# CederGroupHub/smol

Hardware: AMD Instinct MI355X
Metric: attempted MC flips/s (node) + ns/flip/replica, 4096-site FCC canonical (higher is better)
Workload: dtype f64

## Files before the change

### smol_amd/csrc/mc_lean.h

```cpp
#pragma once
#include "smolmc_common.h"

template <int CTRL> __device__ __forceinline__ double dpp_xor_add(double v) {
    const int lo = __builtin_amdgcn_update_dpp(__double2loint(v), __double2loint(v), CTRL, 0xf, 0xf, true);
    const int hi = __builtin_amdgcn_update_dpp(__double2hiint(v), __double2hiint(v), CTRL, 0xf, 0xf, true);
    return v + __hiloint2double(hi, lo);
}
__device__ __forceinline__ double wave_sum_all(double v) {
    v = dpp_xor_add<0xB1>(v);
    v = dpp_xor_add<0x4E>(v);
    v = dpp_xor_add<0x141>(v);
    v = dpp_xor_add<0x140>(v);
    {
        const unsigned lo = (unsigned)__double2loint(v), hi = (unsigned)__double2hiint(v);
        const auto a = __builtin_amdgcn_permlane16_swap(lo, lo, false, false);
        const auto b = __builtin_amdgcn_permlane16_swap(hi, hi, false, false);
        v = __hiloint2double((int)b[0], (int)a[0]) + __hiloint2double((int)b[1], (int)a[1]);
    }
    {
        const unsigned lo = (unsigned)__double2loint(v), hi = (unsigned)__double2hiint(v);
        const auto a = __builtin_amdgcn_permlane32_swap(lo, lo, false, false);
        const auto b = __builtin_amdgcn_permlane32_swap(hi, hi, false, false);
        v = __hiloint2double((int)b[0], (int)a[0]) + __hiloint2double((int)b[1], (int)a[1]);
    }
    return v;
}

template <int CTRL> __device__ __forceinline__ float dpp_add_f32(float v) {
    const int t = __builtin_amdgcn_update_dpp(0, __float_as_int(v), CTRL, 0xf, 0xf, true);
    return v + __int_as_float(t);
}
__device__ __forceinline__ float wave_sum_f32_uniform(float v) {
    v = dpp_add_f32<0xB1>(v);
    v = dpp_add_f32<0x4E>(v);
    v = dpp_add_f32<0x141>(v);
    v = dpp_add_f32<0x140>(v);
    float total;
    asm volatile("s_nop 1\n\t"
                 "v_add_f32_dpp %1, %1, %1 row_bcast:15 row_mask:0xa bank_mask:0xf\n\t"
                 "s_nop 1\n\t"
                 "v_add_f32_dpp %1, %1, %1 row_bcast:31 row_mask:0xc bank_mask:0xf\n\t"
                 "s_nop 1\n\t"
                 "v_readlane_b32 %0, %1, 63\n\t"
                 "s_nop 1"
                 : "=s"(total), "+v"(v));
    return total;
}
__device__ __forceinline__ float wave_sum_f32_lane63(float v) {
    v = dpp_add_f32<0xB1>(v);
    v = dpp_add_f32<0x4E>(v);
    v = dpp_add_f32<0x141>(v);
    v = dpp_add_f32<0x140>(v);
    asm volatile("s_nop 1\n\t"
                 "v_add_f32_dpp %0, %0, %0 row_bcast:15 row_mask:0xa bank_mask:0xf\n\t"
                 "s_nop 1\n\t"
                 "v_add_f32_dpp %0, %0, %0 row_bcast:31 row_mask:0xc bank_mask:0xf"
                 : "+v"(v));
    return v;
}

__device__ __forceinline__ double lean_ewald_partial(const LeanParams &P, const uint8_t *occ, int lane,
                                                     int s, int swa, int swm, int swb) {
    const double *g = P.ew_G + (size_t)s * P.ew_nact;
    const int W = P.ew_W, na = P.ew_nact;
    double out = 0;
    for (int j0 = lane; j0 < na; j0 += 64 * 8) {
        int k[8];
        double gk[8], q[8];
#pragma unroll
        for (int u = 0; u < 8; ++u) {
            const int jj = min(j0 + 64 * u, na - 1);
            k[u] = P.ew_act[jj];
            gk[u] = g[jj];
        }
#pragma unroll
        for (int u = 0; u < 8; ++u)
            q[u] = P.ew_qs[(size_t)k[u] * W + (int)occ[lean_swz(k[u], swa, swm, swb)]];
#pragma unroll
        for (int u = 0; u < 8; ++u)
            out = fma((j0 + 64 * u < na && k[u] != s) ? q[u] : 0.0, gk[u], out);
    }
    return out;
}

template <int FOOT = 2, bool PRE = false>
__device__ __forceinline__ void field_apply(const LeanParams &P, double *phi, int lane, int s, double dq,
                                            const uint32_t (&e0)[27], const bool have_e0) {
    const int js = s - P.sbase;
    const double keep = phi[js];
    const LeanParamsKernarg Q = rare_params();
    const unsigned char *gx = (const unsigned char *)Q->ew_gx;
    if (gx != nullptr) {
        const uint32_t *E8 = Q->ew_E8;
        const uint32_t s8[1] = {Q->ew_S8[js]};
        const double d[1] = {dq};
        if (PRE && have_e0) field_sweep_gx_pre27(phi, E8, gx, lane, P.ew_nact, s8, d, e0);
        else field_sweep_gx_multi<1, FOOT>(phi, E8, gx, lane, P.ew_nact, s8, d);
    } else {
        const double *g = P.ew_G + (size_t)s * P.ew_nact;
        field_sweep<false>(phi, g, g, lane, P.ew_nact, dq, 0.0);
    }
    phi[js] = keep;
}

template <int FOOT = 2>
__device__ __forceinline__ void field_apply(const LeanParams &P, double *phi, int lane, int s, double dq) {
    const uint32_t none[27] = {};
    field_apply<FOOT, false>(P, phi, lane, s, dq, none, false);
}

template <int FOOT = 1, bool FEW = false>
__device__ __forceinline__ void field_apply_flips(double *phi, int lane, int nfl, int vsite, double vdq) {
    const LeanParamsKernarg Q = rare_params();

    const unsigned char *gx = (const unsigned char *)Q->ew_gx;
    auto site_of = [&](int f) { return (int)rdlane((uint32_t)vsite, f); };
    auto dq_of = [&](int f) {
        return __hiloint2double((int)rdlane((uint32_t)__double2hiint(vdq), f), (int)rdlane((uint32_t)__double2loint(vdq), f));
    };
    const int sb = Q->sbase, na = Q->ew_nact;
    if (gx == nullptr) {
        const double *G = Q->ew_G;
        for (int f = 0; f < nfl; ++f) {
            const double dqf = dq_of(f);
            if (dqf == 0.0) continue;
            const double *g = G + (size_t)site_of(f) * na;
            field_sweep<false>(phi, g, g, lane, na, dqf, 0.0);
        }
        return;
    }
    const uint32_t *E8 = Q->ew_E8, *S8 = Q->ew_S8;
    for (int f0 = 0; f0 < nfl; f0 += 4) {
        const int n = min(4, nfl - f0);
        uint32_t s8[4];
        double dq[4];
#pragma unroll
        for (int k = 0; k < 4; ++k) {
            const int f = k < n ? f0 + k : f0;
            s8[k] = S8[site_of(f) - sb];
            dq[k] = k < n ? dq_of(f) : 0.0;
        }
        if (FEW && n <= 3) {
            const uint32_t a[3] = {s8[0], s8[1], s8[2]};
            const double d[3] = {dq[0], dq[1], dq[2]};
            field_sweep_gx_multi<3, FOOT>(phi, E8, gx, lane, na, a, d);
        } else if (n == 1) {
            const uint32_t a[1] = {s8[0]};
            const double d[1] = {dq[0]};
            field_sweep_gx_multi<1, FOOT>(phi, E8, gx, lane, na, a, d);
        } else if (n == 2) {
            const uint32_t a[2] = {s8[0], s8[1]};
            const double d[2] = {dq[0], dq[1]};
            field_sweep_gx_multi<2, FOOT>(phi, E8, gx, lane, na, a, d);
        } else if (n == 3) {
// ... 155 lines not shown
    static_assert(KF == 0 || (!WL && !BIAS && !SOLO), "correlation-function tables: plain Metropolis layouts only");
    static_assert(!REPLAY || (!WL && OCC == 0), "replay: Metropolis variants (Wang-Landau: mc_wl_kernel)");
    constexpr int NACC = KF ? KF : 1;
    constexpr int EWM = EWX & 3;
    constexpr bool WMU = (EWX & 4) != 0;
    static_assert(!WMU || (HAS_MU && !WL && !REPLAY), "per-walker chemical potentials: semigrand Metropolis variants");
    constexpr bool ROWS = lean_rows(MM);
    constexpr int MMX = lean_mm_max(MM);
    constexpr bool STRAIGHT = ROWS && STEP == SMOLMC_STEP_SWAP && OCC == 0 && !HAS_MU;
    constexpr int TAIL_AHEAD = (STRAIGHT && MM == 21) ? 1 : 0;
    static_assert(!ROWS || (SOLO && NSLOT == 2 && EWX == 0 && !REPLAY && KF == 0 && !WL && !BIAS), "solo rows: plain Metropolis, solo layout");
    constexpr bool HAS_EW = EWM != 0, ew_field = EWM == 2;
    extern __shared__ __attribute__((aligned(16))) unsigned char smem[];
    if ((uint32_t)(uintptr_t)smem != 0u) __builtin_trap();
    const int lane = threadIdx.x & 63;
    const int wave = SOLO ? 0 : threadIdx.x >> 6;
    const int nwaves = SOLO ? 1 : blockDim.x >> 6;
    const int r = uni(blockIdx.x * nwaves + wave);
    const size_t per_wave = (size_t)P.Nlds + 64 * 8 + (WL ? (size_t)P.wl.L * 24 : 0) +
                            ((HAS_EW && ew_field) ? 64 + (size_t)P.ew_nact * 8 : 0);
    double *s_dt = SOLO ? (double *)(smem + ((per_wave + 15) & ~(size_t)15)) : (double *)smem;
    const uint32_t dt_off = SOLO ? (uint32_t)((per_wave + 15) & ~(size_t)15) : 0u;
    double *s_mu = s_dt + P.dt_len;
    double *s_q = s_mu + 8, *s_dg = s_mu + 16;
    unsigned char *wbase = SOLO ? smem : (unsigned char *)(s_mu + 24) + (size_t)wave * per_wave;
    uint8_t *occ = wbase;
    double *s_feat = (double *)(wbase + P.Nlds);
    double *wl_S = s_feat + 64;
    long long *wl_Hh = (long long *)(wl_S + (WL ? P.wl.L : 0));
    long long *wl_Oc = wl_Hh + (WL ? P.wl.L : 0);
    double *phi = (double *)(wbase + P.Nlds + 64 * 8 + 64);
    const int swa = P.swz_a, swm = P.swz_m, swb = P.swz_b;
    for (int i = threadIdx.x; i < P.dt_len; i += blockDim.x) s_dt[i] = P.dt[i];
    if (HAS_MU && !WMU && threadIdx.x < 8) s_mu[threadIdx.x] = threadIdx.x < P.ncodes ? P.mu_row[threadIdx.x] : 0.0;
    if (WMU) {
        s_mu = (double *)(smem + P.mu_cell_off) + uni(wave * 8);
        if (lane < 8 && r < P.R) s_mu[lane] = lane < P.ncodes ? P.mu_row[(size_t)r * 8 + lane] : 0.0;
    }
    if (HAS_EW && ew_field && threadIdx.x < 8) {
        s_q[threadIdx.x] = P.ew_qrow[threadIdx.x];
        s_dg[threadIdx.x] = P.ew_dgrow[threadIdx.x];
    }
    const bool live = r < P.R;
    if (live) {
        const uint32_t *src = (const uint32_t *)(P.occ + (size_t)r * P.Npad);
        for (int i = lane; i < P.Npad / 4; i += 64)
            *(uint32_t *)(occ + lean_swz(4 * i, swa, swm, swb)) = src[i];
        s_feat[lane] = (WL && lane < P.F) ? P.features[(size_t)r * P.F + lane] : 0.0;
        if (HAS_EW && ew_field)
            for (int j = lane; j < P.ew_nact; j += 64) phi[j] = P.ew_phi[(size_t)r * P.ew_nact + j];
        if (WL)
            for (int i = lane; i < P.wl.L; i += 64) {
                wl_S[i] = P.wl.entropy[(size_t)r * P.wl.L + i];
                wl_Hh[i] = P.wl.hist[(size_t)r * P.wl.L + i];
                wl_Oc[i] = P.wl.occur[(size_t)r * P.wl.L + i];
            }
    }
    __syncthreads();
    if (!live) return;

    constexpr bool EPRE = HAS_EW && STEP == SMOLMC_STEP_FLIP && !REPLAY;
    uint32_t ereg[27] = {};
    bool epre_on = false;
    if (EPRE) {
        const LeanParamsKernarg Q = rare_params();
        const uint32_t *E8 = Q->ew_E8;
        epre_on = ew_field && Q->ew_gx != nullptr && (Q->ew_nact >> 6) >= 27;
        if (epre_on) {
#pragma unroll
            for (int u = 0; u < 27; ++u) ereg[u] = E8[64 * u + lane];
        }
    }

    uint32_t doff8[NSLOT], st8[NSLOT][MMX], sfeat[NSLOT];
    double wgt[NSLOT], acc[NSLOT], sfs[NSLOT];
    double accK[NSLOT][NACC];
    uint32_t kslot[NSLOT];
#pragma unroll
    for (int it = 0; it < NSLOT; ++it) {
        const LeanSlot sl = P.slots[it * 64 + lane];
        doff8[it] = sl.doff8 + dt_off;
        sfeat[it] = sl.feat;
        sfs[it] = sl.live ? sl.fs : 0.0;
        kslot[it] = sl.live;
#pragma unroll
        for (int m = 0; m < (ROWS ? lean_mm_of(MM, it) : MM); ++m) st8[it][m] = sl.stride8[m];
        wgt[it] = sl.w;
        acc[it] = 0.0;
#pragma unroll
        for (int k = 0; k < NACC; ++k) accK[it][k] = 0.0;
    }
    const int wl_stride = WL ? P.F : 64;
    const int wl_k = WL ? max(1, min(8, 63 / max(wl_stride, 1))) : 1;
    uint32_t sfeat_wl[NSLOT];
#pragma unroll
    for (int it = 0; it < NSLOT; ++it) sfeat_wl[it] = sfeat[it] + (uint32_t)((lane % wl_k) * wl_stride);
    int wl_rd[8];
#pragma unroll
    for (int k = 0; k < 8; ++k) wl_rd[k] = (WL && k < wl_k && lane < wl_stride) ? lane + k * wl_stride : 63;
    auto wl_cur_feat = [&]() -> double {
        const int f = lane < wl_stride ? lane : 0;
        double t[8];
#pragma unroll
        for (int k = 0; k < 8; ++k) t[k] = k < wl_k ? s_feat[f + (k < wl_k ? k : 0) * wl_stride] : 0.0;
        return ((t[0] + t[1]) + (t[2] + t[3])) + ((t[4] + t[5]) + (t[6] + t[7]));
    };
    auto reduce_features = [&](double *dst) {
#pragma unroll
        for (int it = 0; it < NSLOT; ++it) {
            if (KF == 0) {
                __hip_atomic_fetch_add(&dst[sfeat[it]], sfs[it] * acc[it], __ATOMIC_RELAXED,
                                       __HIP_MEMORY_SCOPE_WAVEFRONT);
            } else {
#pragma unroll
                for (int k = 0; k < NACC; ++k) {
                    const bool on = (uint32_t)k < kslot[it];
                    __hip_atomic_fetch_add(&dst[sfeat[it] + (on ? k : 0)], on ? sfs[it] * accK[it][k] : 0.0,
                                           __ATOMIC_RELAXED, __HIP_MEMORY_SCOPE_WAVEFRONT);
                }
            }
        }
    };
    double H = P.enthalpy[r];
    const double nbeta = WL ? 0.0 : -P.beta[r];
    double wl_m = WL ? P.wl.m[r] : 0.0;
    double wl_bq = WL ? floordiv_exact(H - P.wl.vmin, P.wl.bin) : 0.0;
    const double wl_inv_bin = WL ? 1.0 / P.wl.bin : 0.0;
    long long wl_counter = WL ? P.wl.counter[r] : 0;
    long long wl_rem_check = WL ? (P.wl.check ? wl_counter % P.wl.check : 1) : 0;
    unsigned long long step = P.nsteps[r];
    uint32_t nacc_add = 0;
    const uint32_t key0 = (uint32_t)P.seeds[r], key1 = (uint32_t)(P.seeds[r] >> 32);
    const uint32_t nact = (uint32_t)P.nact, nt8 = P.nt8, snt8 = P.snt8;
    const int sbase = P.sbase;
    double acc_mu = 0.0, acc_ew = 0.0;
    const int btype = BIAS ? P.bias_type : 0;
    const int brows = (btype && btype != SMOLMC_BIAS_FUGACITY) ? P.bias_rows : 0;
    double bias_acc = 0.0, chg[SMOLMC_MAX_BIAS_ROWS];
#pragma unroll
    for (int k = 0; k < SMOLMC_MAX_BIAS_ROWS; ++k) chg[k] = k < brows ? P.charge[(size_t)r * SMOLMC_MAX_BIAS_ROWS + k] : 0.0;
    constexpr bool FAST = !WL && !HAS_EW;
    float thr_lo = 0.0f, thr_hi = 0.0f;
    const double inv_nbeta = FAST ? 1.0 / nbeta : 0.0;
    uint32_t nacc_before = 0;
    int nsite = 0, naddr = 0;
    double *featp = P.features + (size_t)r * P.F;
    const double base_feat = lane < P.F ? featp[lane] : 0.0;
    uint32_t smp_countdown = P.smp.every ? (uint32_t)P.smp.every : 0xffffffffu;
    long long smp_index = 0;
    uint32_t W0 = 0;
    int cand[4] = {0, 0, 0, 0}, canda[4] = {0, 0, 0, 0};
    double vGc = 0.0;
    double logu = 0.0;
    unsigned long long batch64_base = ~0ull;
    unsigned long long batch_base = ~0ull;
    constexpr int ROW = lean_row_len(MM, NSLOT);
    constexpr int NW = SOLO ? ROW : ROW / 2;
    constexpr uint32_t ENT = SOLO ? 4u : 2u;
    constexpr uint32_t SITE_BYTES = 64u * ROW * ENT;
    const __amdgpu_buffer_rsrc_t idx_rs = __builtin_amdgcn_make_buffer_rsrc(
        SOLO ? (void *)P.idx32 : (void *)P.idx, 0, 0x7fffffff, 0x00020000);
    const uint32_t lane_voff = (uint32_t)lane * (ROW * ENT);

    int s1, a1;
    RowWords<NW> row1;
    uint32_t ridx = 0;
    double lu_rp = 0.0;
    int rp_bad = 0;
    auto rp_site = [&](const uint32_t i) -> int {
        const int v = uni(P.rp_steps[((size_t)r * (uint32_t)P.steps + i) * 4]);
        return v >= 0 ? v : sbase;
    };
    {
        if (REPLAY) {
            s1 = rp_site(0u);
        } else {
            const unsigned long long sp = step - 1ull;
            const uint32_t w = (uint32_t)uni((int)philox4x32_10((uint32_t)sp, (uint32_t)(sp >> 32), 0u, 0u,
                                                                key0, key1).w[1]);
            s1 = sbase + (int)__umulhi(w, nact);
        }
        a1 = lean_swz(s1, swa, swm, swb);
        row1 = load_row<NW>(idx_rs, lane_voff, (uint32_t)(ROWS ? a1 : s1) * SITE_BYTES);
    }

    double *wl_pend = WL ? P.wl.meanf + (size_t)r * P.wl.L * P.F : nullptr;
    double wl_pc[8] = {0.0, 0.0, 0.0, 0.0, 0.0, 0.0, 0.0, 0.0};
    auto wl_pend_sum = [&]() -> double {
        return ((wl_pc[0] + wl_pc[1]) + (wl_pc[2] + wl_pc[3])) + ((wl_pc[4] + wl_pc[5]) + (wl_pc[6] + wl_pc[7]));
    };
    uint32_t steps_left = (uint32_t)P.steps;
    while (steps_left != 0u) {
        const unsigned long long base = step & ~15ull;
        if (!REPLAY && base != batch_base) {
            batch_base = base;
            const unsigned long long st = base + (unsigned)(lane >> 2);
            const philox_out o = philox4x32_10((uint32_t)st, (uint32_t)(st >> 32), (uint32_t)(lane & 3),
                                               0u, key0, key1);
            W0 = o.w[0];
            nsite = sbase + (int)__umulhi(o.w[1], nact);
            naddr = lean_swz(nsite, swa, swm, swb);
            if ((step & ~63ull) != batch64_base) {
                batch64_base = step & ~63ull;
                const unsigned long long s64 = batch64_base + (unsigned)lane;
                const philox_out a = philox4x32_10((uint32_t)s64, (uint32_t)(s64 >> 32), 0u, 0u, key0, key1);
                logu = log(philox_u53(a.w[2], a.w[3]));
                if (FAST) {
                    const double thr = logu * inv_nbeta;
                    const double eps = P.fast_eps + 1e-6 * fabs(thr);
                    thr_lo = P.fast_eps > 0.0 ? (float)(thr - eps) : -INFINITY;
                    thr_hi = P.fast_eps > 0.0 ? (float)(thr + eps) : INFINITY;
                }
            }
            if (STEP == SMOLMC_STEP_SWAP) {
                cand[0] = sbase + (int)__umulhi(o.w[0], nact);
                cand[1] = sbase + (int)__umulhi(o.w[1], nact);
                cand[2] = sbase + (int)__umulhi(o.w[2], nact);
                cand[3] = sbase + (int)__umulhi(o.w[3], nact);
#pragma unroll
                for (int j = 0; j < 4; ++j) canda[j] = lean_swz(cand[j], swa, swm, swb);
                if (HAS_EW && ew_field) {
                    const int prev = __shfl(nsite, (lane & ~3) - 4);
                    const int site_l = lane < 4 ? s1 : prev;
                    vGc = P.ew_G[(size_t)cand[0] * P.ew_nact + (site_l - sbase)];
                }
            }
        }
        uint32_t chunk = 16u - (uint32_t)(step & 15ull);
        chunk = min(chunk, steps_left);
        chunk = min(chunk, smp_countdown);
        steps_left -= chunk;
        smp_countdown -= chunk;
        const unsigned long long chunk_end = step + chunk;
        int l4 = (int)(step & 15ull) * 4;
        int l64 = (int)(step & 63ull);
        float tlo_s = 0.0f, thi_s = 0.0f;
        uint32_t va2 = 0u, okm = 0u;
        do {
        __builtin_amdgcn_s_setprio(1);
        int s1n, a1n;
        int rq1 = 0, rq2 = -1, rq3 = 0;
        bool rp_empty = false;
        if (REPLAY) {
            const int *rec = P.rp_steps + ((size_t)r * (uint32_t)P.steps + ridx) * 4;
            const int q0 = uni(rec[0]);
            rq1 = uni(rec[1]); rq2 = uni(rec[2]); rq3 = uni(rec[3]);
            rp_empty = q0 < 0;
            double u = uni_d(P.rp_u[(size_t)r * (uint32_t)P.steps + ridx]);
            if (u != u) u = 0.0;
            lu_rp = log(u);
            s1n = ridx + 1u < (uint32_t)P.steps ? rp_site(ridx + 1u) : s1;
            a1n = lean_swz(s1n, swa, swm, swb);
            if (FAST) {
                const double thr = lu_rp * inv_nbeta, eps = P.fast_eps + 1e-6 * fabs(thr);
                thr_lo = P.fast_eps > 0.0 ? (float)(thr - eps) : -INFINITY;
                thr_hi = P.fast_eps > 0.0 ? (float)(thr + eps) : INFINITY;
            }
        } else {
            s1n = (int)rdlane((uint32_t)nsite, l4);
            a1n = (int)rdlane((uint32_t)naddr, l4);
        }
        if constexpr (STRAIGHT) {
            tlo_s = __uint_as_float(rdlane(__float_as_uint(thr_lo), l64));
            thi_s = __uint_as_float(rdlane(__float_as_uint(thr_hi), l64));
        }
        uint32_t va1 = (uint32_t)a1;
        asm volatile("" : "+v"(va1));
        const int vo1 = (int)occ_ld<SOLO>(occ, va1);
        const int o1 = uni(vo1);
        int nfl, s2, a2, n1, n2 = 0, o2 = 0;
        if (STEP != SMOLMC_STEP_SWAP) { s2 = s1; a2 = a1; }
        int fb = -1;
        if (REPLAY) {
            if (STEP == SMOLMC_STEP_FLIP) {
                nfl = rp_empty ? 0 : 1;
                n1 = rp_empty ? o1 : rq1;
                rp_bad |= (rq2 >= 0) ? 1 : 0;
            } else if (!rp_empty && rq2 >= 0) {
                nfl = 2;
                s2 = rq2;
                a2 = lean_swz(s2, swa, swm, swb);
                o2 = uni((int)occ_ld<SOLO>(occ, (uint32_t)a2));
                n2 = rq3;
                n1 = rq1;
                rp_bad |= (n2 != o1 || n1 != o2) ? 1 : 0;
                n2 = o1; n1 = o2;
            } else {
                nfl = 0; s2 = s1; a2 = a1; o2 = o1; n2 = o1; n1 = o1;
                rp_bad |= (!rp_empty || rq2 >= 0) ? 1 : 0;
            }
        } else if (STEP == SMOLMC_STEP_FLIP) {
            const uint32_t kk = __umulhi(rdlane(W0, l4 + 1), (uint32_t)(P.ncodes - 1));
            n1 = (int)kk + ((int)kk >= o1 ? 1 : 0);
            nfl = 1;
        } else {
            nfl = 2;
            n2 = o1;
#define SMOLMC_CAND_MASK(J)                                                                        \
    const int v##J = (int)occ_ld<SOLO>(occ, (uint32_t)canda[J]);                                   \
    const unsigned long long m##J = __ballot(v##J != o1) & (0xEull << l4);
#define SMOLMC_CAND_TAKE(J)                                                                        \
    {                                                                                              \
        const int b = __ffsll((long long)m##J) - 1;                                                \
        s2 = (int)rdlane((uint32_t)cand[J], b);                                                    \
        a2 = (int)rdlane((uint32_t)canda[J], b);                                                   \
        o2 = (int)rdlane((uint32_t)v##J, b);                                                       \
        if (J == 0) fb = b;                                                                        \
    }
            SMOLMC_CAND_MASK(0)
            if constexpr (STRAIGHT) {
                unsigned long long mt = m0;
                uint32_t ta = (uint32_t)canda[0];
                int tv = v0;
                if (__builtin_expect(m0 == 0ull, 0)) {
                    SMOLMC_CAND_MASK(1)
                    mt = m1; ta = (uint32_t)canda[1]; tv = v1;
                    if (m1 == 0ull) {
                        SMOLMC_CAND_MASK(2)
                        mt = m2; ta = (uint32_t)canda[2]; tv = v2;
                        if (m2 == 0ull) {
                            SMOLMC_CAND_MASK(3)
                            mt = m3; ta = (uint32_t)canda[3]; tv = v3;
                            if (m3 == 0ull) {
                                mt = 1ull; ta = va1; tv = o1; nfl = 0;
                                const unsigned long long cur = chunk_end - chunk;
                                for (uint32_t q = 0;; ++q) {
                                    const philox_out o = philox4x32_10((uint32_t)cur, (uint32_t)(cur >> 32),
                                                                       4u + 64u * q + (uint32_t)lane, 0u, key0, key1);
                                    int selsite = -1, selv = 0;
#pragma unroll
                                    for (int j = 3; j >= 0; --j) {
                                        const int cs = sbase + (int)__umulhi(o.w[j], nact);
                                        const int v = (int)occ[lean_swz(cs, swa, swm, swb)];
                                        if (v != o1) { selsite = lean_swz(cs, swa, swm, swb); selv = v; }
                                    }
                                    const unsigned long long m = __ballot(selsite >= 0);
                                    if (m) {
                                        const int b = __ffsll((long long)m) - 1;
                                        ta = rdlane((uint32_t)selsite, b);
                                        tv = (int)rdlane((uint32_t)selv, b);
                                        nfl = 2;
                                        break;
                                    }
                                    if ((q & 63u) == 0) {
                                        int any = 0;
                                        for (uint32_t a = lane; a < nact; a += 64)
                                            any |= ((int)occ[lean_swz(sbase + (int)a, swa, swm, swb)] != o1);
                                        if (__ballot(any) == 0ull) break;
                                    }
                                }
                            }
                        }
                    }
                }
                const int b = __ffsll((long long)mt) - 1;
                a2 = (int)rdlane(ta, b);
                o2 = (int)rdlane((uint32_t)tv, b);
                s2 = a2;
            } else
            if (m0) SMOLMC_CAND_TAKE(0)
            else {
                SMOLMC_CAND_MASK(1)
                if (m1) SMOLMC_CAND_TAKE(1)
                else {
                    SMOLMC_CAND_MASK(2)
                    if (m2) SMOLMC_CAND_TAKE(2)
                    else {
                        SMOLMC_CAND_MASK(3)
                        if (m3) SMOLMC_CAND_TAKE(3)
                        else {
                            bool hit = false;
                            const unsigned long long cur = chunk_end - chunk;
                            for (uint32_t q = 0;; ++q) {
                                const philox_out o = philox4x32_10((uint32_t)cur, (uint32_t)(cur >> 32),
                                                                   4u + 64u * q + (uint32_t)lane, 0u, key0, key1);
                                int selsite = -1, selv = 0;
#pragma unroll
                                for (int j = 3; j >= 0; --j) {
                                    const int cs = sbase + (int)__umulhi(o.w[j], nact);
                                    const int v = (int)occ[lean_swz(cs, swa, swm, swb)];
                                    if (v != o1) { selsite = ROWS ? lean_swz(cs, swa, swm, swb) : cs; selv = v; }
                                }
                                const unsigned long long m = __ballot(selsite >= 0);
                                if (m) {
                                    const int b = __ffsll((long long)m) - 1;
                                    s2 = (int)rdlane((uint32_t)selsite, b);
                                    a2 = ROWS ? s2 : lean_swz(s2, swa, swm, swb);
                                    o2 = (int)rdlane((uint32_t)selv, b);
                                    hit = true;
                                    break;
                                }
                                if ((q & 63u) == 0) {
                                    int any = 0;
                                    for (uint32_t a = lane; a < nact; a += 64)
                                        any |= ((int)occ[lean_swz(sbase + (int)a, swa, swm, swb)] != o1);
                                    if (__ballot(any) == 0ull) break;
                                }
                            }
                            if (!hit) { nfl = 0; s2 = s1; a2 = a1; o2 = o1; }
                        }
                    }
                }
            }
#undef SMOLMC_CAND_MASK
#undef SMOLMC_CAND_TAKE
            n1 = o2;
        }

        __builtin_amdgcn_s_setprio(2);
        RowWords<NW> row2 = row1;
        if (STEP == SMOLMC_STEP_SWAP) {
            row2 = load_row<NW>(idx_rs, lane_voff, (uint32_t)(ROWS ? a2 : s2) * SITE_BYTES);
        }
        if (WL) {
            unsafeAtomicAdd(wl_pend + lane, wl_pend_sum());
        }

        constexpr bool DIFF = STEP == SMOLMC_STEP_SWAP;
        double e = 0.0, d1[NSLOT], d2[NSLOT];
        uint32_t dp[NSLOT];
        uint32_t ad1[NSLOT], ad2[NSLOT];
        {
            const uint32_t pair1 = (uint32_t)o1 * snt8 + (uint32_t)n1 * nt8;
#pragma unroll
            for (int it = 0; it < NSLOT; ++it) {
                uint32_t a = doff8[it];
                if (DIFF) a = dp[it] = doff8[it] + pair1;
#pragma unroll
                for (int m = 0; m < (ROWS ? lean_mm_of(MM, it) : MM); ++m) a += __umul24(st8[it][m], (uint32_t)occ_ld<SOLO>(occ, bounded(row_addr<SOLO, NW>(row1, (ROWS ? lean_row_off(MM, it) : it * MM) + m), (uint32_t)P.Nlds)));
                if (DIFF) {
                    d1[it] = SMOLMC_LDS_F64(a);
                    if (KF) ad1[it] = a;
                } else {
                    d1[it] = SMOLMC_LDS_F64(a + pair1);
                    if (KF) ad1[it] = a + pair1;
                    e = fma(wgt[it], d1[it], e);
                }
            }
        }
        row1 = load_row<NW>(idx_rs, lane_voff, (uint32_t)(ROWS ? a1n : s1n) * SITE_BYTES);
        double ew_part = 0.0, ew_uni = 0.0;
        double dq1 = 0.0, dq2 = 0.0;
        if (HAS_EW) {
            if (ew_field) {
                dq1 = s_q[n1] - s_q[o1];
                ew_uni = 2.0 * dq1 * phi[s1 - sbase] + (s_dg[n1] - s_dg[o1]);
            } else {
                const int W = P.ew_W;
                dq1 = P.ew_qs[(size_t)s1 * W + n1] - P.ew_qs[(size_t)s1 * W + o1];
                ew_part = 2.0 * dq1 * lean_ewald_partial(P, occ, lane, s1, swa, swm, swb);
                ew_uni = 2.0 * dq1 * P.ew_frozen[s1] +
                         (P.ew_dg[(size_t)s1 * W + n1] - P.ew_dg[(size_t)s1 * W + o1]);
            }
        }
        if (STEP == SMOLMC_STEP_SWAP) {
            occ_st<SOLO>(occ, va1, (uint8_t)n1);
            const uint32_t pair2 = (uint32_t)o2 * snt8 + (uint32_t)n2 * nt8;
            if constexpr (TAIL_AHEAD != 0) {
                uint32_t g[NSLOT][MMX];
#pragma unroll
                for (int it = 0; it < NSLOT; ++it) {
#pragma unroll
                    for (int m = 0; m < lean_mm_of(MM, it); ++m) g[it][m] = (uint32_t)occ_ld<SOLO>(occ, bounded(row_addr<SOLO, NW>(row2, lean_row_off(MM, it) + m), (uint32_t)P.Nlds));
                }
                __builtin_amdgcn_sched_barrier(0);
                l4 = (int)opaque_u32((uint32_t)l4 + 4u);
                l64 = (int)opaque_u32((uint32_t)l64 + 1u);
                chunk = opaque_u32(chunk - 1u);
                va2 = (uint32_t)a2;
                asm volatile("" : "+v"(va2));
                __builtin_amdgcn_sched_barrier(0);
#pragma unroll
                for (int it = 0; it < NSLOT; ++it) {
                    uint32_t a = dp[it];
#pragma unroll
                    for (int m = 0; m < lean_mm_of(MM, it); ++m) a += __umul24(st8[it][m], g[it][m]);
                    d1[it] -= SMOLMC_LDS_F64(a);
                    e = fma(wgt[it], d1[it], e);
                }
            } else
#pragma unroll
            for (int it = 0; it < NSLOT; ++it) {
                uint32_t a = DIFF ? dp[it] : doff8[it];
#pragma unroll
                for (int m = 0; m < (ROWS ? lean_mm_of(MM, it) : MM); ++m) a += __umul24(st8[it][m], (uint32_t)occ_ld<SOLO>(occ, bounded(row_addr<SOLO, NW>(row2, (ROWS ? lean_row_off(MM, it) : it * MM) + m), (uint32_t)P.Nlds)));
                if (DIFF) {
                    d1[it] -= SMOLMC_LDS_F64(a);
                    if (KF) ad2[it] = a;
                    e = fma(wgt[it], d1[it], e);
                } else {
                    d2[it] = SMOLMC_LDS_F64(a + pair2);
                    if (KF) ad2[it] = a + pair2;
                    e = fma(wgt[it], d2[it], e);
                }
            }
            if (HAS_EW) {
                if (ew_field) {
                    dq2 = s_q[n2] - s_q[o2];
                    const double cross =
                        fb >= 0 ? __hiloint2double((int)rdlane((uint32_t)__double2hiint(vGc), fb),
                                                   (int)rdlane((uint32_t)__double2loint(vGc), fb))
                                : P.ew_G[(size_t)s2 * P.ew_nact + (s1 - sbase)];
                    ew_uni += 2.0 * dq2 * (phi[s2 - sbase] + dq1 * cross) + (s_dg[n2] - s_dg[o2]);
                } else {
                    const int W = P.ew_W;
                    dq2 = P.ew_qs[(size_t)s2 * W + n2] - P.ew_qs[(size_t)s2 * W + o2];
                    ew_part += 2.0 * dq2 * lean_ewald_partial(P, occ, lane, s2, swa, swm, swb);
                    ew_uni += 2.0 * dq2 * P.ew_frozen[s2] +
                              (P.ew_dg[(size_t)s2 * W + n2] - P.ew_dg[(size_t)s2 * W + o2]);
                }
            }
        }
        double dMu = 0.0;
        if (HAS_MU && nfl >= 1) {
            dMu = s_mu[n1] - s_mu[o1];
            if (nfl == 2) dMu += s_mu[n2] - s_mu[o2];
        }
        double dH = 0.0, dEw = 0.0;
        double wl_nbq = 0.0;
        double dB = 0.0, dQ[SMOLMC_MAX_BIAS_ROWS] = {0.0, 0.0, 0.0, 0.0};
        if (btype && nfl >= 1) {
            if (btype == SMOLMC_BIAS_FUGACITY) {
                dB = P.bias_pair[o1 * 8 + n1];
                if (nfl == 2) dB += P.bias_pair[o2 * 8 + n2];
            } else {
                double sq_new = 0.0, sq_old = 0.0;
#pragma unroll
                for (int k = 0; k < SMOLMC_MAX_BIAS_ROWS; ++k)
                    if (k < brows) {
                        const double *bp = P.bias_pair + k * P.bias_row_stride;
                        double x = bp[o1 * 8 + n1];
                        if (nfl == 2) x += bp[o2 * 8 + n2];
                        dQ[k] = x;
                        const double cn = chg[k] + x;
                        sq_old += chg[k] * chg[k];
                        sq_new += cn * cn;
                    }
                dB = -P.bias_pen * sq_new - (-P.bias_pen * sq_old);
            }
        }
        auto exact_decision = [&]() -> bool {
            dH = wave_sum_all(e);
            if (HAS_EW) {
                dEw = (ew_field ? 0.0 : wave_sum_all(ew_part)) + ew_uni;
                dH += P.ew_coef * dEw;
            }
            if (HAS_MU) dH -= dMu;
            const double lu = REPLAY ? lu_rp
                                     : __hiloint2double((int)rdlane((uint32_t)__double2hiint(logu), l64 - TAIL_AHEAD),
                                                        (int)rdlane((uint32_t)__double2loint(logu), l64 - TAIL_AHEAD));
            if (!WL) {
                const double exponent = nbeta * dH + 0.0 + dB;
                return __ballot((exponent >= 0.0) || (exponent > lu)) != 0ull;
            } else {
                const double new_h = H + dH;
                if (new_h < P.wl.vmin || new_h >= P.wl.vmax) {
                    return false;
                } else {
                    const int b = (int)wl_bq;
                    wl_nbq = floordiv_exact_inv(new_h - P.wl.vmin, P.wl.bin, wl_inv_bin);
                    const int nb = (int)wl_nbq;
                    const double exponent = wl_S[b] - wl_S[nb] + 0.0;
                    return __ballot((exponent >= 0.0) || (exponent > lu)) != 0ull;
                }
            }
        };
        constexpr bool SELACC = DIFF && FAST && !BIAS;
        uint32_t sel_hi = 0u;
        auto on_accept = [&]() {
            if (KF) {
                const unsigned char *kb = (const unsigned char *)P.dtk;
#pragma unroll
                for (int it = 0; it < NSLOT; ++it) {
                    const uint32_t g1 = doff8[it] * (uint32_t)(SMOLMC_LEAN_MAX_KF - 1) + ad1[it];
                    const uint32_t g2 = doff8[it] * (uint32_t)(SMOLMC_LEAN_MAX_KF - 1) + ad2[it];
#pragma unroll
                    for (int k = 0; k < NACC; ++k) {
                        const bool on = (uint32_t)k < kslot[it];
                        const uint32_t off = (uint32_t)k * P.ktab8;
                        double v = on ? *(const double *)(kb + (g1 + off)) : 0.0;
                        if (STEP == SMOLMC_STEP_SWAP) {
                            const double v2 = on ? *(const double *)(kb + (g2 + off)) : 0.0;
                            v = DIFF ? v - v2 : v + v2;
                        }
                        accK[it][k] += v;
                    }
                }
            }
            if (SELACC) {
                sel_hi = 0x3ff00000u;
            } else if (!WL) {
#pragma unroll
                for (int it = 0; it < NSLOT; ++it) acc[it] += d1[it];
                if (STEP == SMOLMC_STEP_SWAP && !DIFF) {
#pragma unroll
                    for (int it = 0; it < NSLOT; ++it) acc[it] += d2[it];
                }
            } else {
#pragma unroll
                for (int it = 0; it < NSLOT; ++it) {
                    const double dd = (STEP == SMOLMC_STEP_SWAP && !DIFF) ? d1[it] + d2[it] : d1[it];
                    __hip_atomic_fetch_add(&s_feat[sfeat_wl[it]], sfs[it] * dd, __ATOMIC_RELAXED,
                                           __HIP_MEMORY_SCOPE_WAVEFRONT);
                }
            }
            if (STEP == SMOLMC_STEP_FLIP) occ_st<SOLO>(occ, va1, (uint8_t)n1);
            if (STEP == SMOLMC_STEP_SWAP) occ_st<SOLO>(occ, (uint32_t)a2, (uint8_t)(ROWS ? vo1 : n2));
            if (HAS_EW && ew_field) {
                if (STEP == SMOLMC_STEP_SWAP) {
                    if (dq1 != 0.0 || dq2 != 0.0) field_apply2(P, phi, lane, s1, dq1, s2, dq2);
                } else if (dq1 != 0.0) {
                    field_apply<2, EPRE>(P, phi, lane, s1, dq1, ereg, epre_on);
                }
            }
            acc_mu += dMu;
            acc_ew += dEw;
            bias_acc += dB;
#pragma unroll
            for (int k = 0; k < SMOLMC_MAX_BIAS_ROWS; ++k) chg[k] += dQ[k];
            if (!FAST) H += dH;
            if (!SELACC) nacc_add++;
        };
        auto on_reject = [&]() {
            if (STEP == SMOLMC_STEP_SWAP) {
            occ_st<SOLO>(occ, va1, (uint8_t)(ROWS ? vo1 : o1));
            }
        };
        nacc_before = nacc_add;
        bool accepted = false;
        __builtin_amdgcn_s_setprio(3);
        if (FAST && !BIAS) {
            const float ef = (float)((HAS_MU && lane == 0) ? e - dMu : e);
            if constexpr (STRAIGHT) {
                const float Sv = wave_sum_f32_lane63(ef);
                const uint32_t ha = opaque_u32((uint32_t)(__ballot(Sv < tlo_s) >> 32));
                const uint32_t hr = opaque_u32((uint32_t)(__ballot(Sv > thi_s) >> 32));
                okm = (uint32_t)((int)ha >> 31);
                if (__builtin_expect((int)(ha | hr) >= 0, 0)) okm = 0u - (uint32_t)uni((int)exact_decision());
                okm = opaque_u32(okm);
                sel_hi = okm & 0x3ff00000u;
                uint32_t vst = (uint32_t)vo1;
                asm("" : "+v"(vst));
                const uint32_t vb = TAIL_AHEAD ? va2 : (uint32_t)a2;
                occ_st<SOLO>(occ, (vb & okm) | (va1 & ~okm), (uint8_t)vst);
            } else {
            const float S = wave_sum_f32_uniform(ef);
            const unsigned long long bit = 1ull << (REPLAY ? 0 : l64);
            const bool ca = (__ballot(S < thr_lo) & bit) != 0ull;
            const bool cr = (__ballot(S > thr_hi) & bit) != 0ull;
            if (ca) on_accept();
            else if (cr) on_reject();
            else if (exact_decision()) on_accept();
            else on_reject();
            }
        } else {
            accepted = exact_decision();
            if (accepted) on_accept();
            else on_reject();
        }
        if (SELACC) {
            const uint32_t sh = (uint32_t)uni((int)sel_hi);
            const double sel = __hiloint2double((int)sh, 0);
#pragma unroll
            for (int it = 0; it < NSLOT; ++it) acc[it] = fma(sel, d1[it], acc[it]);
            if constexpr (STRAIGHT) nacc_add -= okm;
            else
            nacc_add += sh >> 29;
        }
        s1 = s1n;
        a1 = a1n;
        __builtin_amdgcn_s_setprio(0);
        if (REPLAY) {
            double lane_e = 0.0;
            if (FAST) {
#pragma unroll
                for (int it = 0; it < NSLOT; ++it) lane_e = fma(wgt[it], acc[it], lane_e);
            }
            const double Hnow = FAST ? H + (wave_sum_all(lane_e) - acc_mu) : H;
            if (lane == 0) {
                const size_t k = (size_t)r * (uint32_t)P.steps + ridx;
                P.rp_acc[k] = (uint8_t)(nacc_add != nacc_before);
                P.rp_H[k] = Hnow;
            }
            ridx++;
        }

        if (WL) {
            const double bq = accepted ? wl_nbq : wl_bq;
            wl_bq = bq;
            if (bq >= 0.0 && bq < (double)P.wl.L) {
                const int b = (int)bq;
                wl_counter++;
                if (++wl_rem_check == P.wl.check) wl_rem_check = 0;
                wl_pend = P.wl.meanf + ((size_t)r * P.wl.L + b) * P.F;
#pragma unroll
                for (int k = 0; k < 8; ++k) wl_pc[k] = s_feat[wl_rd[k]];
                if (lane == 0) {
                    __hip_atomic_fetch_add(&wl_S[b], wl_m, __ATOMIC_RELAXED, __HIP_MEMORY_SCOPE_WAVEFRONT);
                    __hip_atomic_fetch_add(&wl_Hh[b], 1ll, __ATOMIC_RELAXED, __HIP_MEMORY_SCOPE_WAVEFRONT);
                    __hip_atomic_fetch_add(&wl_Oc[b], 1ll, __ATOMIC_RELAXED, __HIP_MEMORY_SCOPE_WAVEFRONT);
                }
            }
            if (wl_rem_check == 0) {
                const LeanParamsKernarg Q = rare_params();
                wl_m = wl_flatness_check(wl_S, wl_Hh, Q->wl.L, Q->wl.flat, Q->wl.div, wl_m, lane);
            }
        }

        if constexpr (!TAIL_AHEAD) {
        l4 += 4;
        l64 += 1;
        --chunk;
        }
        } while (chunk != 0u);
        step = chunk_end;

        if (smp_countdown == 0) {
            const LeanParamsKernarg Q = rare_params();
            const int qF = Q->F, qFce = Q->Fce;
            double *const q_feat = Q->smp.feat;
            smp_countdown = (uint32_t)Q->smp.every;
            const size_t row = (size_t)smp_index * Q->R + r;
            smp_index++;
            if (WL) {
                const double fcur = wl_cur_feat();
                if (lane < qF) q_feat[row * qF + lane] = fcur;
            } else {
                s_feat[lane] = 0.0;
                reduce_features(s_feat);
                if (lane < qFce) q_feat[row * qF + lane] = base_feat + s_feat[lane];
            }
            if (!WL && HAS_EW && lane == qFce) q_feat[row * qF + lane] = base_feat + acc_ew;
            if (!WL && HAS_MU && lane == qFce + (HAS_EW ? 1 : 0))
                q_feat[row * qF + lane] = base_feat + acc_mu;
            double lane_e = 0.0;
            if (FAST) {
#pragma unroll
                for (int it = 0; it < NSLOT; ++it) lane_e = fma(wgt[it], acc[it], lane_e);
            }
            const double Hnow = FAST ? H + (wave_sum_all(lane_e) - acc_mu) : H;
            if (lane == 0) {
                Q->smp.H[row] = Hnow;
                Q->smp.acc[row] = (uint8_t)(nacc_add != nacc_before);
                if (BIAS && Q->smp_bias_off) (Q->smp.H + Q->smp_bias_off)[row] = Q->bias[r] + bias_acc;
            }
            if (Q->smp.occ) {
                const int qNpad = Q->Npad;
                uint32_t *dst = (uint32_t *)(Q->smp.occ + row * qNpad);
                for (int i = lane; i < qNpad / 4; i += 64)
                    dst[i] = *(const uint32_t *)(occ + lean_swz(4 * i, swa, swm, swb));
            }
        }
    }

    if (HAS_EW && ew_field)
        for (int j = lane; j < P.ew_nact; j += 64) P.ew_phi[(size_t)r * P.ew_nact + j] = phi[j];
    {
        uint32_t *dst = (uint32_t *)(P.occ + (size_t)r * P.Npad);
        for (int i = lane; i < P.Npad / 4; i += 64)
            dst[i] = *(const uint32_t *)(occ + lean_swz(4 * i, swa, swm, swb));
    }
    if (WL) {
        const double fcur = wl_cur_feat();
        unsafeAtomicAdd(wl_pend + lane, wl_pend_sum());
        if (lane < P.F) featp[lane] = fcur;
        for (int i = lane; i < P.wl.L; i += 64) {
            P.wl.entropy[(size_t)r * P.wl.L + i] = wl_S[i];
            P.wl.hist[(size_t)r * P.wl.L + i] = wl_Hh[i];
            P.wl.occur[(size_t)r * P.wl.L + i] = wl_Oc[i];
        }
        if (lane == 0) {
            P.wl.m[r] = wl_m;
            P.wl.counter[r] = wl_counter;
        }
    } else {
        s_feat[lane] = 0.0;
        reduce_features(s_feat);
        if (lane < P.Fce) featp[lane] = base_feat + s_feat[lane];
    }
    if (FAST) {
        double lane_e = 0.0;
#pragma unroll
        for (int it = 0; it < NSLOT; ++it) lane_e = fma(wgt[it], acc[it], lane_e);
        H += wave_sum_all(lane_e) - acc_mu;
    }
    if (btype && lane == 0) {
        P.bias[r] += bias_acc;
#pragma unroll
        for (int k = 0; k < SMOLMC_MAX_BIAS_ROWS; ++k)
            if (k < brows) P.charge[(size_t)r * SMOLMC_MAX_BIAS_ROWS + k] = chg[k];
    }
// ... 1130 lines not shown
```

### smol_amd/csrc/probe_sweeps.hip

```cpp
#include "smolmc_common.h"

thread_local std::string smolmc_g_err;

#define SMOLMC_PROBE_GUARD 128
#define SMOLMC_PROBE_SLACK (27 * 64)

enum ProbeVariant {
    PV_MULTI_1_2 = 0,
    PV_MULTI_1_1,
    PV_MULTI_1_0,
    PV_MULTI_2_1,
    PV_MULTI_2_0,
    PV_MULTI_3_1,
    PV_MULTI_3_0,
    PV_MULTI_4_1,
    PV_MULTI_4_0,
    PV_MULTI_4_M1,
    PV_PRE27,
    PV_GROUPS_1_16,
    PV_GROUPS_2_16,
    PV_DENSE_1,
    PV_DENSE_2,
    PV_DENSE_1_6,
    PV_DENSE_2_4,
    PV_COUNT
};

struct ProbeFlips {
    uint32_t s8[4];
    double dq[4];
};

template <int NF, int FOOT>
__device__ __forceinline__ void probe_multi(double *phi, const uint32_t *E8, const unsigned char *gx, int lane, int na,
                                            const ProbeFlips &F) {
    uint32_t s8[NF];
    double dq[NF];
#pragma unroll
    for (int f = 0; f < NF; ++f) {
        s8[f] = F.s8[f];
        dq[f] = F.dq[f];
    }
    field_sweep_gx_multi<NF, FOOT>(phi, E8, gx, lane, na, s8, dq);
}

template <int NF>
__device__ __forceinline__ void probe_groups16(double *phi, const uint32_t *E8, const unsigned char *gx, int lane,
                                               const ProbeFlips &F) {
    uint32_t e0w[16];
#pragma unroll
    for (int u = 0; u < 16; ++u) e0w[u] = E8[64 * u + lane];
    uint32_t s8[NF];
    double dq[NF];
#pragma unroll
    for (int f = 0; f < NF; ++f) {
        s8[f] = F.s8[f];
        dq[f] = F.dq[f];
    }
    field_sweep_gx_groups<NF, 16>(phi + lane, e0w, gx, s8, dq, 0);
}

template <int V>
__device__ __forceinline__ void probe_sweep(double *phi, const uint32_t *E8, const unsigned char *gx, const double *ga,
                                            const double *gb, int lane, int na, const ProbeFlips &F) {
    if (V == PV_MULTI_1_2) probe_multi<1, 2>(phi, E8, gx, lane, na, F);
    if (V == PV_MULTI_1_1) probe_multi<1, 1>(phi, E8, gx, lane, na, F);
    if (V == PV_MULTI_1_0) probe_multi<1, 0>(phi, E8, gx, lane, na, F);
    if (V == PV_MULTI_2_1) probe_multi<2, 1>(phi, E8, gx, lane, na, F);
    if (V == PV_MULTI_2_0) probe_multi<2, 0>(phi, E8, gx, lane, na, F);
    if (V == PV_MULTI_3_1) probe_multi<3, 1>(phi, E8, gx, lane, na, F);
    if (V == PV_MULTI_3_0) probe_multi<3, 0>(phi, E8, gx, lane, na, F);
    if (V == PV_MULTI_4_1) probe_multi<4, 1>(phi, E8, gx, lane, na, F);
    if (V == PV_MULTI_4_0) probe_multi<4, 0>(phi, E8, gx, lane, na, F);
    if (V == PV_MULTI_4_M1) probe_multi<4, -1>(phi, E8, gx, lane, na, F);
    if (V == PV_PRE27) {
        uint32_t e0[27];
#pragma unroll
        for (int u = 0; u < 27; ++u) e0[u] = E8[64 * u + lane];
        const uint32_t s8[1] = {F.s8[0]};
        const double dq[1] = {F.dq[0]};
        field_sweep_gx_pre27(phi, E8, gx, lane, na, s8, dq, e0);
    }
    if (V == PV_GROUPS_1_16) probe_groups16<1>(phi, E8, gx, lane, F);
    if (V == PV_GROUPS_2_16) probe_groups16<2>(phi, E8, gx, lane, F);
    if (V == PV_DENSE_1) field_sweep<false>(phi, ga, ga, lane, na, F.dq[0], 0.0);
    if (V == PV_DENSE_2) field_sweep<true>(phi, ga, gb, lane, na, F.dq[0], F.dq[1]);
    if (V == PV_DENSE_1_6) field_sweep<false, 6>(phi, ga, ga, lane, na, F.dq[0], 0.0);
    if (V == PV_DENSE_2_4) field_sweep<true, 4>(phi, ga, gb, lane, na, F.dq[0], F.dq[1]);
}

template <int V, bool LDS>
__global__ __launch_bounds__(64) void probe_kernel(double *phi_all, const long long *phi_off, const long long *tab_off,
                                                   const int *na_list, const uint32_t *E8_all, const unsigned char *gx,
                                                   const double *ga_all, const double *gb_all, ProbeFlips F) {
    extern __shared__ double s_phi[];
    const int b = blockIdx.x, lane = threadIdx.x;
    const int na = na_list[b];
    double *slice = phi_all + phi_off[b];
    const uint32_t *E8 = E8_all ? E8_all + tab_off[b] : nullptr;
    const double *ga = ga_all ? ga_all + tab_off[b] : nullptr, *gb = gb_all ? gb_all + tab_off[b] : nullptr;
    double *phi = slice;
    if (LDS) {
        for (int j = lane; j < na + SMOLMC_PROBE_GUARD; j += 64) s_phi[j] = slice[j];
        __syncthreads();
        phi = s_phi;
    }
    probe_sweep<V>(phi, E8, gx, ga, gb, lane, na, F);
    if (LDS) {
        __syncthreads();
        for (int j = lane; j < na + SMOLMC_PROBE_GUARD; j += 64) slice[j] = s_phi[j];
    }
}

template <int V>
static hipError_t probe_launch(bool lds, int nblocks, int na_max, double *phi_all, const long long *phi_off,
                               const long long *tab_off, const int *na_list, const uint32_t *E8_all, const unsigned char *gx,
                               const double *ga_all, const double *gb_all, const ProbeFlips &F, hipStream_t stream) {
    if (lds) {
        const size_t bytes = (size_t)(na_max + SMOLMC_PROBE_GUARD + SMOLMC_PROBE_SLACK) * sizeof(double);
        hipLaunchKernelGGL((probe_kernel<V, true>), dim3(nblocks), dim3(64), bytes, stream, phi_all, phi_off, tab_off, na_list,
                           E8_all, gx, ga_all, gb_all, F);
    } else {
        hipLaunchKernelGGL((probe_kernel<V, false>), dim3(nblocks), dim3(64), 0, stream, phi_all, phi_off, tab_off, na_list,
                           E8_all, gx, ga_all, gb_all, F);
    }
    return hipGetLastError();
}

extern "C" {

int smolmc_probe_variant_count(void) { return PV_COUNT; }
int smolmc_probe_guard(void) { return SMOLMC_PROBE_GUARD; }

int smolmc_probe_sweep(int variant, int lds, int nblocks, int na_min, int na_max, double *phi_all, const long long *phi_off,
                       const long long *tab_off, const int *na_list, const uint32_t *E8_all, const unsigned char *gx,
                       const double *ga_all, const double *gb_all, const uint32_t *s8, const double *dq) {
    if (variant < 0 || variant >= PV_COUNT || nblocks <= 0 || na_min < 1 || na_max < na_min) return -1;
    const bool dense = variant >= PV_DENSE_1;
    if (!phi_all || !phi_off || !tab_off || !na_list || !s8 || !dq) return -2;
    if (dense ? (!ga_all || !gb_all) : (!E8_all || !gx)) return -2;
    if (variant == PV_PRE27 && na_min < 27 * 64) return -3;
    if ((variant == PV_GROUPS_1_16 || variant == PV_GROUPS_2_16) && (na_min != 1024 || na_max != 1024)) return -3;
    if (lds && (size_t)(na_max + SMOLMC_PROBE_GUARD + SMOLMC_PROBE_SLACK) * sizeof(double) > 64 * 1024) return -4;
    ProbeFlips F;
    for (int f = 0; f < 4; ++f) {
        F.s8[f] = s8[f];
        F.dq[f] = dq[f];
    }
    hipError_t e = hipSuccess;
#define PROBE_CASE(V)                                                                                                      \
    case V:                                                                                                                \
        e = probe_launch<V>(lds != 0, nblocks, na_max, phi_all, phi_off, tab_off, na_list, E8_all, gx, ga_all, gb_all, F, 0); \
        break;
    switch (variant) {
        PROBE_CASE(PV_MULTI_1_2)
        PROBE_CASE(PV_MULTI_1_1)
        PROBE_CASE(PV_MULTI_1_0)
        PROBE_CASE(PV_MULTI_2_1)
        PROBE_CASE(PV_MULTI_2_0)
        PROBE_CASE(PV_MULTI_3_1)
        PROBE_CASE(PV_MULTI_3_0)
        PROBE_CASE(PV_MULTI_4_1)
        PROBE_CASE(PV_MULTI_4_0)
        PROBE_CASE(PV_MULTI_4_M1)
        PROBE_CASE(PV_PRE27)
        PROBE_CASE(PV_GROUPS_1_16)
        PROBE_CASE(PV_GROUPS_2_16)
        PROBE_CASE(PV_DENSE_1)
        PROBE_CASE(PV_DENSE_2)
        PROBE_CASE(PV_DENSE_1_6)
        PROBE_CASE(PV_DENSE_2_4)
    }
#undef PROBE_CASE
    if (e != hipSuccess) return (int)e;
    e = hipDeviceSynchronize();
    return (int)e;
}

}
```

Baseline: 20.25 billion.

## Derive fast accept thresholds per step from batch Philox words with hardware log2

In the STRAIGHT path, each lane's fast-accept thresholds now come from the per-16-step Philox output word w2. They use a single-precision hardware log2 bracketed by interval bounds, replacing the separate 64-step Philox batch and double-precision log. The exact uniform log is computed only when the threshold test is ambiguous, which removes the per-lane l64 index bookkeeping and a Philox call. The risk is that the float bracketing must stay conservative so decisions match the exact path. It also changes the random stream used for acceptance, and adds probe kernels to check threshold and log2 accuracy.

```diff
diff --git a/smol_amd/csrc/mc_lean.h b/smol_amd/csrc/mc_lean.h
--- a/smol_amd/csrc/mc_lean.h
+++ b/smol_amd/csrc/mc_lean.h
@@ -1,5 +1,6 @@
 #pragma once
 #include "smolmc_common.h"
+#include "rows_thresholds.h"
 
 template <int CTRL> __device__ __forceinline__ double dpp_xor_add(double v) {
     const int lo = __builtin_amdgcn_update_dpp(__double2loint(v), __double2loint(v), CTRL, 0xf, 0xf, true);
@@ -461,6 +462,9 @@
     int cand[4] = {0, 0, 0, 0}, canda[4] = {0, 0, 0, 0};
     double vGc = 0.0;
     double logu = 0.0;
+    uint32_t W2 = 0, W3 = 0;
+    const float thr_cf = STRAIGHT ? rows_threshold_scale(inv_nbeta) : 0.0f;
+    const float thr_ef = STRAIGHT ? rows_threshold_eps(P.fast_eps) : 0.0f;
     unsigned long long batch64_base = ~0ull;
     unsigned long long batch_base = ~0ull;
     constexpr int ROW = lean_row_len(MM, NSLOT);
@@ -509,6 +513,11 @@
             W0 = o.w[0];
             nsite = sbase + (int)__umulhi(o.w[1], nact);
             naddr = lean_swz(nsite, swa, swm, swb);
+            if constexpr (STRAIGHT) {
+                W2 = o.w[2];
+                W3 = o.w[3];
+                rows_thresholds(o.w[2], thr_cf, thr_ef, thr_lo, thr_hi);
+            } else
             if ((step & ~63ull) != batch64_base) {
                 batch64_base = step & ~63ull;
                 const unsigned long long s64 = batch64_base + (unsigned)lane;
@@ -570,8 +579,8 @@
             a1n = (int)rdlane((uint32_t)naddr, l4);
         }
         if constexpr (STRAIGHT) {
-            tlo_s = __uint_as_float(rdlane(__float_as_uint(thr_lo), l64));
-            thi_s = __uint_as_float(rdlane(__float_as_uint(thr_hi), l64));
+            tlo_s = __uint_as_float(rdlane(__float_as_uint(thr_lo), l4));
+            thi_s = __uint_as_float(rdlane(__float_as_uint(thr_hi), l4));
         }
         uint32_t va1 = (uint32_t)a1;
         asm volatile("" : "+v"(va1));
@@ -774,7 +783,6 @@
                 }
                 __builtin_amdgcn_sched_barrier(0);
                 l4 = (int)opaque_u32((uint32_t)l4 + 4u);
-                l64 = (int)opaque_u32((uint32_t)l64 + 1u);
                 chunk = opaque_u32(chunk - 1u);
                 va2 = (uint32_t)a2;
                 asm volatile("" : "+v"(va2));
@@ -855,7 +863,7 @@
                 dH += P.ew_coef * dEw;
             }
             if (HAS_MU) dH -= dMu;
-            const double lu = REPLAY ? lu_rp
+            const double lu = (REPLAY || STRAIGHT) ? lu_rp
                                      : __hiloint2double((int)rdlane((uint32_t)__double2hiint(logu), l64 - TAIL_AHEAD),
                                                         (int)rdlane((uint32_t)__double2loint(logu), l64 - TAIL_AHEAD));
             if (!WL) {
@@ -945,7 +953,10 @@
                 const uint32_t ha = opaque_u32((uint32_t)(__ballot(Sv < tlo_s) >> 32));
                 const uint32_t hr = opaque_u32((uint32_t)(__ballot(Sv > thi_s) >> 32));
                 okm = (uint32_t)((int)ha >> 31);
-                if (__builtin_expect((int)(ha | hr) >= 0, 0)) okm = 0u - (uint32_t)uni((int)exact_decision());
+                if (__builtin_expect((int)(ha | hr) >= 0, 0)) {
+                    lu_rp = log(philox_u53(rdlane(W2, l4 - 4 * TAIL_AHEAD), rdlane(W3, l4 - 4 * TAIL_AHEAD)));
+                    okm = 0u - (uint32_t)uni((int)exact_decision());
+                }
                 okm = opaque_u32(okm);
                 sel_hi = okm & 0x3ff00000u;
                 uint32_t vst = (uint32_t)vo1;
diff --git a/smol_amd/csrc/probe_sweeps.hip b/smol_amd/csrc/probe_sweeps.hip
--- a/smol_amd/csrc/probe_sweeps.hip
+++ b/smol_amd/csrc/probe_sweeps.hip
@@ -1,4 +1,5 @@
 #include "smolmc_common.h"
+#include "rows_thresholds.h"
 
 thread_local std::string smolmc_g_err;
 
@@ -178,3 +179,46 @@
 }
 
 }
+
+__global__ __launch_bounds__(256) void probe_rows_thresholds_kernel(const uint32_t *w2, long long n, double beta,
+                                                                    double fast_eps, float *lo, float *hi) {
+    const double nbeta = -beta;
+    const double inv_nbeta = 1.0 / nbeta;
+    const float c_f = rows_threshold_scale(inv_nbeta), eps_f = rows_threshold_eps(fast_eps);
+    for (long long i = blockIdx.x * (long long)blockDim.x + threadIdx.x; i < n; i += (long long)gridDim.x * blockDim.x) {
+        float a, b;
+        rows_thresholds(w2[i], c_f, eps_f, a, b);
+        lo[i] = a;
+        hi[i] = b;
+    }
+}
+
+__global__ __launch_bounds__(256) void probe_rows_log2_kernel(uint32_t first, long long n, int scaled, float *out) {
+    for (long long i = blockIdx.x * (long long)blockDim.x + threadIdx.x; i < n; i += (long long)gridDim.x * blockDim.x)
+        out[i] = rows_log2_hw(first + (uint32_t)i, scaled);
+}
+
+extern "C" {
+
+int smolmc_probe_rows_widen_ulp(void) { return SMOLMC_ROWS_LOG2_WIDEN_ULP; }
+double smolmc_probe_rows_measured_ulp(void) { return (double)SMOLMC_ROWS_LOG2_MEASURED_ULP; }
+
+int smolmc_probe_rows_thresholds(const uint32_t *w2, long long n, double beta, double fast_eps, float *lo, float *hi) {
+    if (!w2 || !lo || !hi || n <= 0) return -1;
+    const int blocks = (int)((n + 255) / 256 < 4096 ? (n + 255) / 256 : 4096);
+    hipLaunchKernelGGL(probe_rows_thresholds_kernel, dim3(blocks), dim3(256), 0, 0, w2, n, beta, fast_eps, lo, hi);
+    hipError_t e = hipGetLastError();
+    if (e != hipSuccess) return (int)e;
+    return (int)hipDeviceSynchronize();
+}
+
+int smolmc_probe_rows_log2(uint32_t first, long long n, int scaled, float *out) {
+    if (!out || n <= 0 || (unsigned long long)first + (unsigned long long)n > (1ull << 24) + 1ull) return -1;
+    const int blocks = (int)((n + 255) / 256 < 4096 ? (n + 255) / 256 : 4096);
+    hipLaunchKernelGGL(probe_rows_log2_kernel, dim3(blocks), dim3(256), 0, 0, first, n, scaled, out);
+    hipError_t e = hipGetLastError();
+    if (e != hipSuccess) return (int)e;
+    return (int)hipDeviceSynchronize();
+}
+
+}
diff --git a/smol_amd/csrc/rows_thresholds.h b/smol_amd/csrc/rows_thresholds.h
--- /dev/null
+++ b/smol_amd/csrc/rows_thresholds.h
@@ -0,0 +1,30 @@
+#pragma once
+#include <stdint.h>
+#include <math.h>
+
+#define SMOLMC_ROWS_LOG2_MEASURED_ULP 1.0f
+#define SMOLMC_ROWS_LOG2_WIDEN_ULP 3
+
+__device__ __forceinline__ float rows_threshold_scale(double inv_nbeta) {
+    return (float)(0.69314718055994530942 * inv_nbeta);
+}
+
+__device__ __forceinline__ float rows_threshold_eps(double fast_eps) {
+    return fast_eps > 0.0 ? (float)(fast_eps * (1.0 + 0x1p-20)) : INFINITY;
+}
+
+__device__ __forceinline__ void rows_thresholds(uint32_t w2, float c_f, float eps_f, float &thr_lo, float &thr_hi) {
+    constexpr float rel = (float)(SMOLMC_ROWS_LOG2_WIDEN_ULP + 2) * 0x1p-23f;
+    const float x = (float)(w2 >> 8);
+    const float u_lo = x * 0x1p-24f;
+    const float u_hi = __builtin_fmaf(x, 0x1p-24f, 0x1p-24f);
+    const float t_hi = __builtin_amdgcn_logf(u_lo) * c_f;
+    const float t_lo = __builtin_amdgcn_logf(u_hi) * c_f;
+    thr_hi = __builtin_fmaf(t_hi, 1.0f + rel, eps_f);
+    thr_lo = __builtin_fmaf(t_lo, 1.0f - rel, -eps_f);
+}
+
+__device__ __forceinline__ float rows_log2_hw(uint32_t m, int scaled) {
+    const float x = (float)m;
+    return __builtin_amdgcn_logf(scaled ? x * 0x1p-24f : x);
+}
```

New measurement: 20.79 billion, median of 6. 1.03x the previous value.
